# kallenordling/cesm_emulator

Measured on NVIDIA B200. Metric: train samples/s (baseline cfg), higher is better.
Workload: dtype fp16

## Files before the change

### cesm_emulator_b200/_lib.py

```python
from __future__ import annotations

import ctypes
from ctypes import POINTER, Structure, c_char_p, c_float, c_int32, c_int64, c_void_p
from pathlib import Path

_PKG = Path(__file__).resolve().parent
_VARIANT = __import__("os").environ.get("CESM_LIB_VARIANT", "")
LIB_PATH = _PKG / (f"libcesm_b200_{_VARIANT}.so" if _VARIANT else "libcesm_b200.so")

CESM_MAX_TAPS = 16


class IgemmArgs(Structure):

    _fields_ = [
        ("a0", c_void_p), ("a1", c_void_p),
        ("c0", c_int32), ("c1", c_int32),
        ("n", c_int32), ("h", c_int32), ("w", c_int32),
        ("stride", c_int32),
        ("num_taps", c_int32),
        ("tap_dh", c_int32 * CESM_MAX_TAPS), ("tap_dw", c_int32 * CESM_MAX_TAPS),
        ("wt", c_void_p), ("cout", c_int32),
        ("oh", c_int32), ("ow", c_int32),
        ("out", c_void_p), ("out_fp32", c_int32), ("ldo", c_int32),
# ... 68 lines not shown
    _lib = lib
    return lib


_P, _I, _L, _F = c_void_p, ctypes.c_int, ctypes.c_longlong, c_float
_SIGNATURES: dict[str, list] = {
    "cesm_igemm": [POINTER(IgemmArgs), _P],
    "cesm_wgrad": [POINTER(WgradArgs), _P],
    "cesm_pack_weight": [_P, _P, _I, _I, _I, _L, _L, POINTER(c_int32), _P],
    "cesm_pack_weights_batched": [_P, _I, _P],
    "cesm_unpack_wgrads_batched": [_P, _I, _P],
    "cesm_unpack_wgrad": [_P, _P, _I, _I, _I, _L, _L, POINTER(c_int32), _I, _P],
    "cesm_adamw_step": [_P, _P, _P, _P, _L, _P, _P, _F, _F, _F, _F, _P],
    "cesm_colsum": [_P, _P, _L, _I, _I, _P],
    "cesm_gn_stats": [_P, _P, _I, _L, _I, _I, _P],
    "cesm_gn_apply_fwd": [_P, _P, _P, _P, _P, _P, _P, _I, _L, _I, _I, _F, _P],
    "cesm_gn_bwd": [_P, _P, _P, _P, _P, _P, _P, _P, _P, _P, _P, _P, _I, _L, _I, _I, _F, _I, _P],
    "cesm_ln_fwd": [_P, _P, _P, _L, _I, _F, _P],
    "cesm_ln_bwd": [_P, _P, _P, _P, _P, _P, _L, _I, _F, _I, _P],
    "cesm_tattn_fwd": [_P, _P, _P, _P, _P, _P, _I, _I, _I, _I, _I, _F, _P],
    "cesm_tattn_bwd": [_P, _P, _P, _P, _P, _P, _P, _P, _P, _I, _I, _I, _I, _I, _F, _P],
    "cesm_tattn_proj_fwd": [_P, _P, _P, _P, _P, _P, _I, _I, _I, _I, _I, _I, _F, _P],
    "cesm_tattn_proj_bwd": [_P, _P, _P, _P, _P, _P, _P, _P, _I, _I, _I, _I, _I, _I, _F, _P],
    "cesm_tattn_long_fwd": [_P, _P, _P, _P, _P, _P, _I, _I, _I, _I, _I, _F, _P],
    "cesm_tattn_long_bwd": [_P, _P, _P, _P, _P, _P, _P, _P, _P, _I, _I, _I, _I, _I, _F, _P],
    "cesm_mattn_fwd": [_P, _P, _P, _I, _I, _I, _I, _F, _P],
    "cesm_mattn_bwd": [_P, _P, _P, _P, _P, _P, _I, _I, _I, _I, _F, _P],
    "cesm_linattn_fwd": [_P, _P, _P, _I, _I, _I, _I, _F, _P],
    "cesm_linattn_fwd_out": [_P, _P, _P, _P, _P, _P, _I, _I, _I, _I, _I, _F, _P],
    "cesm_linattn_bwd": [_P, _P, _P, _P, _P, _I, _I, _I, _I, _F, _P],
    "cesm_film_fwd": [_P, _P, _P, _I, _I, _I, _I, _P],
    "cesm_film_bwd": [_P, _P, _P, _I, _I, _P, _I, _I, _I, _P],
    "cesm_gather_windows": [_P, _P, _P, _P, _P, _I, _I, _I, _I, _I, _I, _I, _I, _P],
    "cesm_qkv_bwd": [_P, _P, _P, _P, _P, _L, _L, _I, _I, _P],
    "cesm_input_patches": [_P, _P, _I, _I, _P, _I, _I, _I, _I, _I, _I, _P],
    "cesm_input_weight_pack": [_P, _P, _P, _I, _I, _I, _P],
    "cesm_input_conv_fwd": [_P, _P, _I, _I, _P, _P, _P, _I, _I, _I, _I, _I, _I, _P],
    "cesm_input_conv_wgrad": [_P, _P, _I, _I, _P, _P, _P, _I, _I, _I, _I, _I, _I, _P],
    "cesm_out_conv_fwd": [_P, _P, _P, _P, _I, _I, _I, _L, _I, _P],
    "cesm_out_conv_bwd": [_P, _P, _P, _P, _P, _P, _I, _I, _I, _L, _I, _P],
    "cesm_sinusoidal": [_P, _P, _I, _I, _P],
    "cesm_small_linear_fwd": [_P, _P, _P, _P, _I, _I, _I, _I, _P],
    "cesm_small_linear_bwd": [_P, _P, _P, _P, _P, _P, _I, _I, _I, _I, _I, _P],
    "cesm_q_sample": [_P, _P, _P, _P, _P, _P, _I, _L, _P],
    "cesm_mse_fwd": [_P, _P, _P, _P, _L, _P],
    "cesm_scale_by_scalar": [_P, _P, _F, _P, _L, _P],
# ... 76 lines not shown
```

### cesm_emulator_b200/csrc/api_common.h

```cpp
#pragma once
#include <cuda.h>
#include <cuda_runtime.h>
#include <stdarg.h>
#include <stdint.h>

#include "../../include/cesm_b200.h"

namespace cesm {

int set_error(int code, const char* fmt, ...);
#define CESM_CHECK_CUDA(expr)                                                                  \
    do {                                                                                       \
        cudaError_t _e = (expr);                                                               \
        if (_e != cudaSuccess)                                                                 \
            return ::cesm::set_error(CESM_ERR_CUDA, "%s failed: %s (%s:%d)", #expr,            \
                                     cudaGetErrorString(_e), __FILE__, __LINE__);              \
    } while (0)
void note_launch();
#define CESM_CHECK_LAUNCH()            \
    do {                               \
        ::cesm::note_launch();         \
        CESM_CHECK_CUDA(cudaGetLastError()); \
    } while (0)
bool scratch_prezeroed();
// ... 30 lines not shown
    cfg.blockDim = block;
    cfg.dynamicSmemBytes = smem;
    cfg.stream = st;
    cudaLaunchAttribute attr[2];
    int n = 0;
    if (pdl_enabled()) {
        attr[n].id = cudaLaunchAttributeProgrammaticStreamSerialization;
        attr[n].val.programmaticStreamSerializationAllowed = 1;
        ++n;
    }
    if (cluster_x > 1) {
        attr[n].id = cudaLaunchAttributeClusterDimension;
        attr[n].val.clusterDim.x = (unsigned)cluster_x;
        attr[n].val.clusterDim.y = 1;
        attr[n].val.clusterDim.z = 1;
        ++n;
    }
    cfg.attrs = attr;
    cfg.numAttrs = n;
    return cudaLaunchKernelEx(&cfg, kern, static_cast<KArgs>(args)...);
}

int get_tensor_map_h16(CUtensorMap* out, const void* base, int rank, const uint64_t* dims,
                        const uint64_t* strides_bytes, const uint32_t* box);

inline cudaStream_t as_stream(void* s) { return reinterpret_cast<cudaStream_t>(s); }
inline int ceil_div(int a, int b) { return (a + b - 1) / b; }

}
```

### cesm_emulator_b200/csrc/api_core.cu

```cuda
#include <stdlib.h>

#include <atomic>
#include <mutex>
#include <string>
#include <unordered_map>

#include "api_common.h"
#include "igemm.h"

namespace cesm {

static thread_local std::string g_last_error;
static std::atomic<long long> g_launches{0};
void note_launch() { g_launches.fetch_add(1, std::memory_order_relaxed); }
bool pdl_enabled() {
    static const bool on = [] { const char* e = getenv("CESM_NO_PDL"); return !(e && atoi(e)); }();
    return on;
}
static std::atomic<int> g_prezeroed{0};
bool scratch_prezeroed() { return g_prezeroed.load(std::memory_order_relaxed) != 0; }

int set_error(int code, const char* fmt, ...) {
    char buf[1024];
    va_list ap;
// ... 2 lines not shown
    va_end(ap);
    g_last_error = buf;
    return code;
}

typedef CUresult (*EncodeTiledFn)(CUtensorMap*, CUtensorMapDataType, cuuint32_t, void*, const cuuint64_t*,
                                  const cuuint64_t*, const cuuint32_t*, const cuuint32_t*, CUtensorMapInterleave,
                                  CUtensorMapSwizzle, CUtensorMapL2promotion, CUtensorMapFloatOOBfill);

static EncodeTiledFn resolve_encode() {
    static EncodeTiledFn fn = nullptr;
    static std::once_flag once;
    std::call_once(once, [] {
        void* p = nullptr;
        cudaDriverEntryPointQueryResult q;
        if (cudaGetDriverEntryPoint("cuTensorMapEncodeTiled", &p, cudaEnableDefault, &q) == cudaSuccess &&
            q == cudaDriverEntryPointSuccess)
            fn = reinterpret_cast<EncodeTiledFn>(p);
    });
    return fn;
}

struct MapKey {
    uint64_t v[14];
    bool operator==(const MapKey& o) const {
        for (int i = 0; i < 14; ++i)
            if (v[i] != o.v[i]) return false;
        return true;
    }
};
struct MapKeyHash {
    size_t operator()(const MapKey& k) const {
        uint64_t h = 1469598103934665603ull;
        for (int i = 0; i < 14; ++i) {
            h ^= k.v[i];
            h *= 1099511628211ull;
        }
        return static_cast<size_t>(h);
    }
};
static std::mutex g_map_mutex;
static std::unordered_map<MapKey, CUtensorMap, MapKeyHash> g_map_cache;

int get_tensor_map_h16(CUtensorMap* out, const void* base, int rank, const uint64_t* dims,
                        const uint64_t* strides_bytes, const uint32_t* box) {
    CESM_REQUIRE(rank >= 2 && rank <= 4, "tensor map rank %d unsupported", rank);
    CESM_REQUIRE((reinterpret_cast<uintptr_t>(base) & 15u) == 0, "tensor base %p not 16-byte aligned", base);
    MapKey key{};
    key.v[0] = reinterpret_cast<uint64_t>(base);
    key.v[1] = static_cast<uint64_t>(rank);
    for (int i = 0; i < rank; ++i) {
        key.v[2 + i] = dims[i];
        key.v[6 + i] = (i == 0) ? 0 : strides_bytes[i - 1];
        key.v[10 + i] = box[i];
    }
    {
        std::lock_guard<std::mutex> lk(g_map_mutex);
        auto it = g_map_cache.find(key);
        if (it != g_map_cache.end()) {
            *out = it->second;
            return CESM_OK;
        }
    }
    EncodeTiledFn enc = resolve_encode();
    if (!enc) return set_error(CESM_ERR_CUDA, "cuTensorMapEncodeTiled unavailable (no CUDA driver?)");
    cuuint64_t gdim[4], gstr[3];
    cuuint32_t bx[4], es[4];
    for (int i = 0; i < rank; ++i) {
        gdim[i] = dims[i];
        bx[i] = box[i];
        es[i] = 1;
        if (i > 0) {
            gstr[i - 1] = strides_bytes[i - 1];
            CESM_REQUIRE(gstr[i - 1] % 16 == 0, "tensor map stride %llu not a multiple of 16 B",
                         (unsigned long long)gstr[i - 1]);
        }
        CESM_REQUIRE(bx[i] >= 1 && bx[i] <= 256, "tensor map box[%d]=%u out of range", i, bx[i]);
    }
    alignas(64) CUtensorMap m;
    CUresult r = enc(&m, CU_TENSOR_MAP_DATA_TYPE_FLOAT16, rank, const_cast<void*>(base), gdim, gstr, bx, es,
                     CU_TENSOR_MAP_INTERLEAVE_NONE, CU_TENSOR_MAP_SWIZZLE_128B, CU_TENSOR_MAP_L2_PROMOTION_L2_256B,
                     CU_TENSOR_MAP_FLOAT_OOB_FILL_NONE);
    if (r != CUDA_SUCCESS) return set_error(CESM_ERR_CUDA, "cuTensorMapEncodeTiled failed with CUresult %d", (int)r);
    {
        std::lock_guard<std::mutex> lk(g_map_mutex);
        if (g_map_cache.size() > 8192) g_map_cache.clear();
        g_map_cache.emplace(key, m);
    }
    *out = m;
    return CESM_OK;
}

static void choose_tile(int n, int oh, int ow, int* bw, int* bh, int* bn) {
    long long best_tiles = -1;
    int b_w = 1, b_h = 1, b_n = 1;
    for (int w = 1; w <= 128 && w <= ow; ++w) {
        if (!(w == ow || (w & (w - 1)) == 0)) continue;
        for (int h = 1; h * w <= 128 && h <= oh; ++h) {
            if (!(h == oh || (h & (h - 1)) == 0)) continue;
            int nn = 128 / (w * h);
            if (nn > n) nn = n;
            if (nn < 1) nn = 1;
            if (w != ow || h != oh) nn = 1;
            long long tiles = 1LL * ceil_div(ow, w) * ceil_div(oh, h) * ceil_div(n, nn);
// ... 584 lines not shown
```

### cesm_emulator_b200/kernels.py

```python
from __future__ import annotations

import ctypes
from typing import Optional, Sequence, Tuple

import torch

from . import _lib
from ._lib import IgemmArgs

H16 = torch.float16


def _stream() -> ctypes.c_void_p:
    return ctypes.c_void_p(torch.cuda.current_stream().cuda_stream)


def _ptr(t: Optional[torch.Tensor]) -> Optional[int]:
    return None if t is None else t.data_ptr()


def _req_cuda(*ts: Optional[torch.Tensor]) -> None:
    for t in ts:
        if t is not None and not t.is_cuda:
            raise _lib.CesmError("cesm_emulator_b200 kernels need CUDA tensors (no CPU fallback)")
# ... 339 lines not shown

def tattn_proj_fwd(xn, wqkv_packed, bias, cs, sn, B: int, F: int, HW: int, H: int, D: int, scale: float):
    _req_cuda(xn, wqkv_packed, bias, cs, sn)
    assert xn.dtype == H16 and wqkv_packed.dtype == H16 and tuple(wqkv_packed.shape) == (3 * H * D, 64)
    rows = B * F * HW
    out = torch.empty((rows, H * D), dtype=H16, device=xn.device)
    _lib.call("cesm_tattn_proj_fwd", _ptr(xn), _ptr(wqkv_packed), _ptr(bias), _ptr(cs), _ptr(sn), _ptr(out), B, F, HW, H, D,
              64, scale, _stream(),
              _meta={"kind": "fused", "flops": 2.0 * rows * 64 * 3 * H * D, "bytes": float(rows * (64 + H * D) * 2)})
    return out


def tattn_proj_bwd(xn, wqkv_packed, bias, cs, sn, dout, B: int, F: int, HW: int, H: int, D: int, scale: float):
    _req_cuda(xn, wqkv_packed, bias, cs, sn, dout)
    rows = B * F * HW
    dqkv = torch.empty((rows, 3 * H * D), dtype=H16, device=xn.device)
    dbias = zero_scratch((H, F, F), xn.device)
    _lib.call("cesm_tattn_proj_bwd", _ptr(xn), _ptr(wqkv_packed), _ptr(bias), _ptr(cs), _ptr(sn), _ptr(dout), _ptr(dqkv),
              _ptr(dbias), B, F, HW, H, D, 64, scale, _stream(),
              _meta={"kind": "fused", "flops": 2.0 * rows * 64 * 3 * H * D, "bytes": float(rows * (64 + H * D + 3 * H * D) * 2)})
    return dqkv, dbias


def mattn_fwd(qkv, NI: int, n: int, H: int, D: int, scale: float):
    _req_cuda(qkv)
    assert qkv.dtype == H16 and qkv.shape == (NI * n, 3 * H * D), (tuple(qkv.shape), NI, n, H, D)
    out = torch.empty((NI * n, H * D), dtype=H16, device=qkv.device)
    lse = torch.empty((NI * n, H), dtype=torch.float32, device=qkv.device)
    _lib.call("cesm_mattn_fwd", _ptr(qkv), _ptr(out), _ptr(lse), NI, n, H, D, scale, _stream(),
              _meta={"kind": "fwd", "flops": 4.0 * NI * H * n * n * D, "bytes": float(qkv.numel() * 2 + out.numel() * 2)})
    return out, lse


def mattn_bwd(qkv, out, lse, dout, NI: int, n: int, H: int, D: int, scale: float):
    _req_cuda(qkv, out, lse, dout)
    assert qkv.dtype == H16 and out.dtype == H16 and dout.dtype == H16 and lse.dtype == torch.float32
    assert qkv.shape == (NI * n, 3 * H * D) and out.shape == dout.shape == (NI * n, H * D) and lse.numel() == NI * n * H
    dqkv = torch.empty_like(qkv)
    delta = torch.empty((NI * n, H), dtype=torch.float32, device=qkv.device)
    _lib.call("cesm_mattn_bwd", _ptr(qkv), _ptr(out), _ptr(lse), _ptr(dout), _ptr(dqkv), _ptr(delta), NI, n, H, D, scale,
              _stream(), _meta={"kind": "bwd", "flops": 14.0 * NI * H * n * n * D,
                                "bytes": float(qkv.numel() * 4 + out.numel() * 2 + dout.numel() * 2)})
    return dqkv


def linattn_fwd(qkv, NI: int, n: int, H: int, D: int, scale: float):
# ... 208 lines not shown
```

### cesm_emulator_b200/ops.py

```python
from __future__ import annotations

import weakref
from typing import Optional, Tuple

import torch

from . import _lib
from . import kernels as K

H16 = torch.float16

_PHASE_TAPS = {0: [(0, 1), (-1, 3)], 1: [(1, 0), (0, 2)]}


_OUTER_GRAD = [True]


class _Fn(torch.autograd.Function):
    @classmethod
    def apply(cls, *args, **kwargs):
        _OUTER_GRAD[0] = torch.is_grad_enabled()
        return super().apply(*args, **kwargs)


# ... 570 lines not shown
        dxn, dw = K.qkv_bwd(dqkv4, xn, wdq)
        return dxn, dw.view_as(wqkv)
    return K.igemm(dqkv4, wdq), _conv_wgrad(wqkv, xn, None, dqkv4, 1)


class TemporalAttnBlockFn(_Fn):

    @staticmethod
    def forward(ctx, x, gamma, wqkv, wout, pos_bias, cs, sn, B, F, meta):
        x = x.contiguous()
        NI, H_, W_, C = x.shape
        heads, D, eps = meta.heads, meta.dim_head, meta.eps
        hidden = heads * D
        g = gamma.reshape(-1)
        pos_bias = pos_bias.contiguous().float()
        train = _train(ctx)
        if F == 1 and not train and C == 64:
            wln, colsum = _fold_f1(meta, wqkv, wout, hidden, C, gamma=gamma)
            return K.igemm(x, wln, residual=x, ln_fold=(colsum, eps))
        xn = K.ln_fwd(x, g, eps)
        if F == 1 and not train:
            return K.igemm(xn, _fold_f1(meta, wqkv, wout, hidden, C), residual=x)
        wq = _conv_fwd_weight(meta.cq, wqkv, 3 * hidden, C, 1, train)
        fused = K.tattn_proj_ok(C, F, H_ * W_, heads, D, train)
        if fused:
            qkv, lse = None, None
            o = K.tattn_proj_fwd(xn.view(-1, C), wq, pos_bias, cs, sn, B, F, H_ * W_, heads, D, D ** -0.5)
        else:
            qkv = K.igemm(xn, wq)
            o, lse = K.tattn_fwd(qkv.view(-1, 3 * hidden), pos_bias, cs, sn, B, F, H_ * W_, heads, D, D ** -0.5)
        y = K.igemm(o.view(NI, H_, W_, hidden), _conv_fwd_weight(meta.co, wout, C, hidden, 1, train), residual=x)
        ctx.wdq = _conv_dgrad_weights(meta.cq, wqkv, 3 * hidden, C, 0, 1, train)[0]
        ctx.wdo = _conv_dgrad_weights(meta.co, wout, C, hidden, 0, 1, train)[0]
        ctx.wq_fwd = wq if fused else None
        saved = [x, g, xn, o, pos_bias, cs, sn, wqkv, wout, gamma]
        if not fused:
            saved.append(qkv)
            if F > 4:
                saved.append(lse)
        ctx.save_for_backward(*saved)
        ctx.cfg, ctx.gshape = (B, F, heads, D, eps), gamma.shape
        return y

    @staticmethod
    def backward(ctx, dy):
        saved = ctx.saved_tensors
        x, g, xn, o, pos_bias, cs, sn, wqkv, wout, gamma = saved[:10]
        qkv = saved[10] if len(saved) > 10 else None
        lse = saved[11] if len(saved) > 11 else None
        B, F, heads, D, eps = ctx.cfg
        hidden = heads * D
        NI, H_, W_, C = x.shape
        dy = dy.contiguous()
        do = K.igemm(dy, ctx.wdo)
        dwout = _conv_wgrad(wout, o.view(NI, H_, W_, hidden), None, dy, 1)
        if ctx.wq_fwd is not None:
            dqkv, dbias = K.tattn_proj_bwd(xn.view(-1, C), ctx.wq_fwd, pos_bias, cs, sn, do.view(-1, hidden), B, F, H_ * W_,
                                           heads, D, D ** -0.5)
        else:
            dqkv, dbias = K.tattn_bwd(qkv.view(-1, 3 * hidden), pos_bias, cs, sn, o if F > 4 else None, lse,
                                      do.view(-1, hidden), B, F, H_ * W_, heads, D, D ** -0.5)
        dqkv4 = dqkv.view(NI, H_, W_, 3 * hidden)
        dxn, dwqkv = _qkv_backward(wqkv, ctx.wdq, xn, dqkv4)
        if _direct_all(gamma):
            dx, _ = K.ln_bwd(x, g, dxn, dy, eps, into=gamma.grad.view(-1))
            _ready(gamma)
            dgamma = None
        else:
            dx, dg = K.ln_bwd(x, g, dxn, dy, eps)
            dgamma = dg.view(ctx.gshape)
        return dx, dgamma, dwqkv, dwout, dbias, None, None, None, None, None


class MidAttnBlockFn(_Fn):

    @staticmethod
    def forward(ctx, x, gamma, wqkv, wout, meta):
        x = x.contiguous()
        NI, H_, W_, C = x.shape
# ... 226 lines not shown
```

### include/cesm_b200.h

```cpp
#ifndef CESM_B200_H
#define CESM_B200_H

#include <stddef.h>
#include <stdint.h>

#ifdef __cplusplus
extern "C" {
#endif

typedef enum cesm_status {
    CESM_OK = 0,
    CESM_ERR_INVALID = -1,
    CESM_ERR_CUDA = -2,
    CESM_ERR_INTERNAL = -3
} cesm_status;

const char* cesm_last_error(void);
const char* cesm_version(void);
long long cesm_launch_count(void);


#define CESM_MAX_TAPS 16

typedef struct cesm_igemm_args {
// ... 73 lines not shown
int cesm_gn_stats(const void* x, float* sums, int B, long long P, int C, int G, void* stream);
int cesm_gn_apply_fwd(const void* x, const float* sums, const float* gamma, const float* beta, const float* film,
                      const void* residual, void* out, int B, long long P, int C, int G, float eps, void* stream);
int cesm_gn_bwd(const void* x, const void* dout, const float* sums, const float* gamma, const float* beta,
                const float* film, float* csum, void* dx, float* dgamma, float* dbeta, float* dfilm,
                float* dconv_bias, int B, long long P, int C, int G, float eps, int accumulate_params, void* stream);

int cesm_ln_fwd(const void* x, const float* gamma, void* out, long long M, int C, float eps, void* stream);
int cesm_ln_bwd(const void* x, const float* gamma, const void* dy, const void* dres, void* dx, float* dgamma,
                long long M, int C, float eps, int accumulate, void* stream);

int cesm_tattn_fwd(const void* qkv, const float* bias, const float* cs, const float* sn, void* out, float* lse,
                   int B, int F, int HW, int H, int dim_head, float scale, void* stream);
int cesm_tattn_bwd(const void* qkv, const float* bias, const float* cs, const float* sn, const void* out,
                   const float* lse, const void* dout, void* dqkv, float* dbias, int B, int F, int HW, int H,
                   int dim_head, float scale, void* stream);

int cesm_tattn_proj_fwd(const void* xn, const void* wqkv, const float* bias, const float* cs, const float* sn, void* out,
                        int B, int F, int HW, int H, int dim_head, int cin, float scale, void* stream);
int cesm_tattn_proj_bwd(const void* xn, const void* wqkv, const float* bias, const float* cs, const float* sn,
                        const void* dout, void* dqkv, float* dbias, int B, int F, int HW, int H, int dim_head, int cin,
                        float scale, void* stream);

int cesm_tattn_long_max_frames(void);
int cesm_tattn_long_fwd(const void* qkv, const float* bias_diag, const float* cs, const float* sn, void* out,
                        float* lse, int B, int F, int HW, int H, int dim_head, float scale, void* stream);
int cesm_tattn_long_bwd(const void* qkv, const float* bias_diag, const float* cs, const float* sn, const void* out,
                        const float* lse, const void* dout, void* dqkv, float* dbias_diag, int B, int F, int HW, int H,
                        int dim_head, float scale, void* stream);

int cesm_mattn_fwd(const void* qkv, void* out, float* lse, int NI, int n, int H, int dim_head, float scale, void* stream);
int cesm_mattn_bwd(const void* qkv, const void* out, const float* lse, const void* dout, void* dqkv, float* delta, int NI,
                   int n, int H, int dim_head, float scale, void* stream);

size_t cesm_linattn_ws_floats(int NI, int H);
int cesm_linattn_fwd(const void* qkv, float* ws, void* out, int NI, int n, int H, int dim_head, float scale,
                     void* stream);
int cesm_linattn_fwd_out(const void* qkv, float* ws, const float* wout, const float* bias, const void* x, void* y, int NI,
                         int n, int H, int dim_head, int C, float scale, void* stream);
int cesm_linattn_bwd(const void* qkv, float* ws, const void* dout, float* scratch, void* dqkv, int NI, int n, int H,
                     int dim_head, float scale, void* stream);

typedef struct cesm_film_desc {
    const float* W;
    const float* bias;
    float* dW;
// ... 43 lines not shown
```

Measured before the change: 188.3.

## Add tcgen05/UMMA fused QKV-projection temporal attention kernels for training

Adds a new warp-specialized Blackwell kernel that computes the QKV projection with tcgen05 UMMA into tensor memory, then applies RoPE, small-frame softmax attention and writes output via TMA, with a matching backward that also accumulates the bias gradient. Training temporal attention with C=64, 8 heads, dim 32 and up to 3 frames now routes here instead of the existing fused proj path. The goal is to remove the separate QKV materialization and use tensor cores for the projection. Tensor map creation gains a 64B swizzle option and the map cache key grows to include it. The new pipeline is complex, and correctness or occupancy depends on the large shared-memory footprint and the 512-column TMEM allocation.

```diff
diff --git a/cesm_emulator_b200/_lib.py b/cesm_emulator_b200/_lib.py
--- a/cesm_emulator_b200/_lib.py
+++ b/cesm_emulator_b200/_lib.py
@@ -114,6 +114,8 @@
     "cesm_tattn_bwd": [_P, _P, _P, _P, _P, _P, _P, _P, _P, _I, _I, _I, _I, _I, _F, _P],
     "cesm_tattn_proj_fwd": [_P, _P, _P, _P, _P, _P, _I, _I, _I, _I, _I, _I, _F, _P],
     "cesm_tattn_proj_bwd": [_P, _P, _P, _P, _P, _P, _P, _P, _I, _I, _I, _I, _I, _I, _F, _P],
+    "cesm_tattn_umma_fwd": [_P, _P, _P, _P, _P, _P, _I, _I, _I, _I, _I, _I, _F, _P],
+    "cesm_tattn_umma_bwd": [_P, _P, _P, _P, _P, _P, _P, _P, _I, _I, _I, _I, _I, _I, _F, _P],
     "cesm_tattn_long_fwd": [_P, _P, _P, _P, _P, _P, _I, _I, _I, _I, _I, _F, _P],
     "cesm_tattn_long_bwd": [_P, _P, _P, _P, _P, _P, _P, _P, _P, _I, _I, _I, _I, _I, _F, _P],
     "cesm_mattn_fwd": [_P, _P, _P, _I, _I, _I, _I, _F, _P],
diff --git a/cesm_emulator_b200/csrc/api_common.h b/cesm_emulator_b200/csrc/api_common.h
--- a/cesm_emulator_b200/csrc/api_common.h
+++ b/cesm_emulator_b200/csrc/api_common.h
@@ -76,7 +76,7 @@
 }
 
 int get_tensor_map_h16(CUtensorMap* out, const void* base, int rank, const uint64_t* dims,
-                        const uint64_t* strides_bytes, const uint32_t* box);
+                        const uint64_t* strides_bytes, const uint32_t* box, int swizzle_bytes = 128);
 
 inline cudaStream_t as_stream(void* s) { return reinterpret_cast<cudaStream_t>(s); }
 inline int ceil_div(int a, int b) { return (a + b - 1) / b; }
diff --git a/cesm_emulator_b200/csrc/api_core.cu b/cesm_emulator_b200/csrc/api_core.cu
--- a/cesm_emulator_b200/csrc/api_core.cu
+++ b/cesm_emulator_b200/csrc/api_core.cu
@@ -48,9 +48,9 @@
 }
 
 struct MapKey {
-    uint64_t v[14];
+    uint64_t v[15];
     bool operator==(const MapKey& o) const {
-        for (int i = 0; i < 14; ++i)
+        for (int i = 0; i < 15; ++i)
             if (v[i] != o.v[i]) return false;
         return true;
     }
@@ -58,7 +58,7 @@
 struct MapKeyHash {
     size_t operator()(const MapKey& k) const {
         uint64_t h = 1469598103934665603ull;
-        for (int i = 0; i < 14; ++i) {
+        for (int i = 0; i < 15; ++i) {
             h ^= k.v[i];
             h *= 1099511628211ull;
         }
@@ -69,8 +69,9 @@
 static std::unordered_map<MapKey, CUtensorMap, MapKeyHash> g_map_cache;
 
 int get_tensor_map_h16(CUtensorMap* out, const void* base, int rank, const uint64_t* dims,
-                        const uint64_t* strides_bytes, const uint32_t* box) {
+                        const uint64_t* strides_bytes, const uint32_t* box, int swizzle_bytes) {
     CESM_REQUIRE(rank >= 2 && rank <= 4, "tensor map rank %d unsupported", rank);
+    CESM_REQUIRE(swizzle_bytes == 128 || swizzle_bytes == 64, "tensor map swizzle %d unsupported", swizzle_bytes);
     CESM_REQUIRE((reinterpret_cast<uintptr_t>(base) & 15u) == 0, "tensor base %p not 16-byte aligned", base);
     MapKey key{};
     key.v[0] = reinterpret_cast<uint64_t>(base);
@@ -80,6 +81,7 @@
         key.v[6 + i] = (i == 0) ? 0 : strides_bytes[i - 1];
         key.v[10 + i] = box[i];
     }
+    key.v[14] = static_cast<uint64_t>(swizzle_bytes);
     {
         std::lock_guard<std::mutex> lk(g_map_mutex);
         auto it = g_map_cache.find(key);
@@ -105,7 +107,8 @@
     }
     alignas(64) CUtensorMap m;
     CUresult r = enc(&m, CU_TENSOR_MAP_DATA_TYPE_FLOAT16, rank, const_cast<void*>(base), gdim, gstr, bx, es,
-                     CU_TENSOR_MAP_INTERLEAVE_NONE, CU_TENSOR_MAP_SWIZZLE_128B, CU_TENSOR_MAP_L2_PROMOTION_L2_256B,
+                     CU_TENSOR_MAP_INTERLEAVE_NONE,
+                     swizzle_bytes == 64 ? CU_TENSOR_MAP_SWIZZLE_64B : CU_TENSOR_MAP_SWIZZLE_128B, CU_TENSOR_MAP_L2_PROMOTION_L2_256B,
                      CU_TENSOR_MAP_FLOAT_OOB_FILL_NONE);
     if (r != CUDA_SUCCESS) return set_error(CESM_ERR_CUDA, "cuTensorMapEncodeTiled failed with CUresult %d", (int)r);
     {
diff --git a/cesm_emulator_b200/csrc/tattn_umma.cu b/cesm_emulator_b200/csrc/tattn_umma.cu
--- /dev/null
+++ b/cesm_emulator_b200/csrc/tattn_umma.cu
@@ -0,0 +1,660 @@
+#include "api_common.h"
+#include "common.cuh"
+
+namespace cesm {
+namespace tu {
+
+static constexpr int C = 64, D = 32, HEADS = 8, HID = HEADS * D, TILE = 128;
+static constexpr int XT = TILE * C * 2;
+static constexpr int WPART = D * C * 2;
+static constexpr int WS = 3 * WPART;
+static constexpr int DOT = TILE * D * 2;
+static constexpr int STT = 32 * D * 2;
+static constexpr int EPI = 256;
+static constexpr uint32_t TM_V = 384;
+
+template <int F, bool BWD>
+struct Cfg {
+    static constexpr int XST = BWD ? 1 : 2;
+    static constexpr int NST = BWD ? 3 * F : F;
+    static constexpr int W_OFF = XST * F * XT;
+    static constexpr int DO_OFF = W_OFF + 2 * WS;
+    static constexpr int ST_OFF = DO_OFF + (BWD ? F * DOT : 0);
+    static constexpr int XB_OFF = ST_OFF + 4 * NST * STT;
+    static constexpr int DB_OFF = XB_OFF + 2 * F * F * TILE * 4;
+    static constexpr int TAB_OFF = DB_OFF + (BWD ? HEADS * F * F * TILE * 4 : 0);
+    static constexpr int BAR_OFF = (TAB_OFF + (2 * F * 16 + HEADS * F * F) * 4 + 7) & ~7;
+    static constexpr int SMEM = 1024 + BAR_OFF + 17 * 8;
+};
+
+struct Maps {
+    CUtensorMap x;
+    CUtensorMap w;
+    CUtensorMap o;
+    CUtensorMap g;
+};
+struct Params {
+    int HW, tiles_per_img, items;
+    float scale;
+    const float* bias;
+    const float* cs;
+    const float* sn;
+    float* dbias;
+};
+
+__device__ __forceinline__ void tma_load_3d(uint32_t dst, const void* map, uint32_t bar, int c0, int c1, int c2) {
+    asm volatile(
+        "cp.async.bulk.tensor.3d.shared::cluster.global.mbarrier::complete_tx::bytes [%0], [%1, {%3, %4, %5}], [%2];"
+        :
+        : "r"(dst), "l"(reinterpret_cast<uint64_t>(map)), "r"(bar), "r"(c0), "r"(c1), "r"(c2)
+        : "memory");
+}
+__device__ __forceinline__ void tma_store_3d(const void* map, uint32_t src, int c0, int c1, int c2) {
+    asm volatile("cp.async.bulk.tensor.3d.global.shared::cta.bulk_group [%0, {%2, %3, %4}], [%1];"
+                 :
+                 : "l"(reinterpret_cast<uint64_t>(map)), "r"(src), "r"(c0), "r"(c1), "r"(c2)
+                 : "memory");
+}
+__device__ __forceinline__ void bulk_commit() { asm volatile("cp.async.bulk.commit_group;" ::: "memory"); }
+__device__ __forceinline__ void bulk_wait_read0() { asm volatile("cp.async.bulk.wait_group.read 0;" ::: "memory"); }
+__device__ __forceinline__ void tmem_ld16(uint32_t taddr, float (&f)[16]) {
+    asm volatile(
+        "tcgen05.ld.sync.aligned.32x32b.x16.b32 "
+        "{%0, %1, %2, %3, %4, %5, %6, %7, %8, %9, %10, %11, %12, %13, %14, %15}, [%16];"
+        : "=f"(f[0]), "=f"(f[1]), "=f"(f[2]), "=f"(f[3]), "=f"(f[4]), "=f"(f[5]), "=f"(f[6]), "=f"(f[7]), "=f"(f[8]),
+          "=f"(f[9]), "=f"(f[10]), "=f"(f[11]), "=f"(f[12]), "=f"(f[13]), "=f"(f[14]), "=f"(f[15])
+        : "r"(taddr)
+        : "memory");
+}
+__device__ __forceinline__ void tmem_ld16(uint32_t taddr, float (&f)[8]) {
+    asm volatile("tcgen05.ld.sync.aligned.32x32b.x8.b32 {%0, %1, %2, %3, %4, %5, %6, %7}, [%8];"
+                 : "=f"(f[0]), "=f"(f[1]), "=f"(f[2]), "=f"(f[3]), "=f"(f[4]), "=f"(f[5]), "=f"(f[6]), "=f"(f[7])
+                 : "r"(taddr)
+                 : "memory");
+}
+template <int N>
+__device__ __forceinline__ void tmem_fence(float (&f)[N]) {
+#pragma unroll
+    for (int i = 0; i < N; ++i) asm volatile("" : "+f"(f[i]));
+}
+__device__ __forceinline__ void sts128(uint32_t addr, uint32_t a, uint32_t b, uint32_t c, uint32_t d) {
+    asm volatile("st.shared.v4.b32 [%0], {%1, %2, %3, %4};" ::"r"(addr), "r"(a), "r"(b), "r"(c), "r"(d) : "memory");
+}
+__device__ __forceinline__ uint4 lds128(uint32_t addr) {
+    uint4 u;
+    asm volatile("ld.shared.v4.b32 {%0, %1, %2, %3}, [%4];"
+                 : "=r"(u.x), "=r"(u.y), "=r"(u.z), "=r"(u.w)
+                 : "r"(addr)
+                 : "memory");
+    return u;
+}
+__device__ __forceinline__ uint32_t sw64(int r, int c) { return r * 64 + ((c ^ ((r >> 1) & 3)) << 4); }
+template <int N>
+__device__ __forceinline__ void put16(uint32_t tile, int r, int c, const float (&f)[N]) {
+#pragma unroll
+    for (int u = 0; u < N / 8; ++u)
+        sts128(tile + sw64(r, (N / 8) * c + u), pack_h2(f[8 * u + 0], f[8 * u + 1]), pack_h2(f[8 * u + 2], f[8 * u + 3]),
+               pack_h2(f[8 * u + 4], f[8 * u + 5]), pack_h2(f[8 * u + 6], f[8 * u + 7]));
+}
+template <int N>
+__device__ __forceinline__ void unpack16(const uint32_t* u, int c, float (&f)[N]) {
+#pragma unroll
+    for (int i = 0; i < N / 2; ++i) {
+        const float2 t = unpack_h2(u[(N / 2) * c + i]);
+        f[2 * i] = t.x;
+        f[2 * i + 1] = t.y;
+    }
+}
+template <int N>
+__device__ __forceinline__ void rope16(float (&f)[N], const float* cs, const float* sn, float scale) {
+#pragma unroll
+    for (int m = 0; m < N / 2; ++m) {
+        const float x0 = f[2 * m] * scale, x1 = f[2 * m + 1] * scale;
+        f[2 * m] = x0 * cs[m] - x1 * sn[m];
+        f[2 * m + 1] = x1 * cs[m] + x0 * sn[m];
+    }
+}
+template <int N>
+__device__ __forceinline__ void rope16_t(float (&f)[N], const float* cs, const float* sn, float scale) {
+#pragma unroll
+    for (int m = 0; m < N / 2; ++m) {
+        const float g0 = f[2 * m], g1 = f[2 * m + 1];
+        f[2 * m] = (g0 * cs[m] + g1 * sn[m]) * scale;
+        f[2 * m + 1] = (g1 * cs[m] - g0 * sn[m]) * scale;
+    }
+}
+template <int N>
+__device__ __forceinline__ float dot16(const float (&a)[N], const float (&b)[N]) {
+    float s = 0.f;
+#pragma unroll
+    for (int i = 0; i < N; ++i) s = fmaf(a[i], b[i], s);
+    return s;
+}
+__device__ __forceinline__ void epi_sync() { asm volatile("bar.sync 5, %0;" ::"n"(EPI) : "memory"); }
+__device__ __forceinline__ void pair_sync(int q) { asm volatile("bar.sync %0, 64;" ::"r"(q + 1) : "memory"); }
+template <int N>
+__device__ __forceinline__ void pair_sum(float (&v)[N], float* xb, int r, int q, int half) {
+    if (half)
+#pragma unroll
+        for (int k = 0; k < N; ++k) xb[k * TILE + r] = v[k];
+    pair_sync(q);
+    if (!half)
+#pragma unroll
+        for (int k = 0; k < N; ++k) {
+            v[k] += xb[k * TILE + r];
+            xb[k * TILE + r] = v[k];
+        }
+    pair_sync(q);
+    if (half)
+#pragma unroll
+        for (int k = 0; k < N; ++k) v[k] = xb[k * TILE + r];
+}
+
+template <int F>
+__device__ __forceinline__ void scores(uint32_t tq, int c2, const float* cs_s, const float* sn_s, float scale, float* s) {
+#pragma unroll
+    for (int i = 0; i < F * F; ++i) s[i] = 0.f;
+#pragma unroll
+    for (int sub = 0; sub < 2; ++sub) {
+        const int c4 = 2 * c2 + sub;
+        float q[F][8], k[F][8];
+#pragma unroll
+        for (int f = 0; f < F; ++f) {
+            tmem_ld16(tq + f * 64 + c4 * 8, q[f]);
+            tmem_ld16(tq + f * 64 + 32 + c4 * 8, k[f]);
+        }
+        tmem_ld_wait();
+#pragma unroll
+        for (int f = 0; f < F; ++f) {
+            tmem_fence(q[f]);
+            tmem_fence(k[f]);
+            rope16(q[f], cs_s + f * 16 + c4 * 4, sn_s + f * 16 + c4 * 4, scale);
+            rope16(k[f], cs_s + f * 16 + c4 * 4, sn_s + f * 16 + c4 * 4, 1.f);
+        }
+#pragma unroll
+        for (int i = 0; i < F; ++i)
+#pragma unroll
+            for (int j = 0; j < F; ++j) s[i * F + j] += dot16(q[i], k[j]);
+    }
+}
+
+template <int F>
+__device__ __forceinline__ void softmax(float* s, const float* bias_s, int h) {
+#pragma unroll
+    for (int i = 0; i < F; ++i) {
+        float m = -INFINITY;
+#pragma unroll
+        for (int j = 0; j < F; ++j) {
+            s[i * F + j] += bias_s[(h * F + i) * F + j];
+            m = fmaxf(m, s[i * F + j]);
+        }
+        float l = 0.f;
+#pragma unroll
+        for (int j = 0; j < F; ++j) {
+            s[i * F + j] = __expf(s[i * F + j] - m);
+            l += s[i * F + j];
+        }
+        const float inv = 1.f / l;
+#pragma unroll
+        for (int j = 0; j < F; ++j) s[i * F + j] *= inv;
+    }
+}
+
+template <int F, bool BWD>
+__device__ __forceinline__ void tattn_umma_body(const Maps& maps, const Params& p) {
+    using K = Cfg<F, BWD>;
+    extern __shared__ uint8_t smem_raw[];
+    const uint32_t smem_base = (smem_u32(smem_raw) + 1023u) & ~1023u;
+    uint8_t* smem_gen = smem_raw + (smem_base - smem_u32(smem_raw));
+    const uint32_t x_base = smem_base, w_base = smem_base + K::W_OFF, do_base = smem_base + K::DO_OFF;
+    const uint32_t bar_base = smem_base + K::BAR_OFF;
+    auto x_full = [&](int s) { return bar_base + 8u * s; };
+    auto x_empty = [&](int s) { return bar_base + 8u * (2 + s); };
+    auto w_full = [&](int s) { return bar_base + 8u * (4 + s); };
+    auto w_empty = [&](int s) { return bar_base + 8u * (6 + s); };
+    auto qk_full = [&](int s) { return bar_base + 8u * (8 + s); };
+    auto qk_empty = [&](int s) { return bar_base + 8u * (10 + s); };
+    const uint32_t v_full = bar_base + 8u * 12, v_empty = bar_base + 8u * 13;
+    const uint32_t do_full = bar_base + 8u * 14, do_empty = bar_base + 8u * 15;
+    const uint32_t tmem_ptr_addr = bar_base + 8u * 16;
+    volatile uint32_t* tmem_ptr_gen = reinterpret_cast<volatile uint32_t*>(smem_gen + (tmem_ptr_addr - smem_base));
+    float* cs_s = reinterpret_cast<float*>(smem_gen + K::TAB_OFF);
+    float* sn_s = cs_s + F * 16;
+    float* bias_s = sn_s + F * 16;
+    float* db_s = reinterpret_cast<float*>(smem_gen + K::DB_OFF);
+    float* xb_s = reinterpret_cast<float*>(smem_gen + K::XB_OFF);
+
+    const int warp = threadIdx.x >> 5, lane = threadIdx.x & 31;
+    if (threadIdx.x == 0) {
+        tma_prefetch_desc(&maps.x);
+        tma_prefetch_desc(&maps.w);
+        tma_prefetch_desc(&maps.o);
+        if (BWD) tma_prefetch_desc(&maps.g);
+        for (int s = 0; s < 2; ++s) {
+            mbar_init(x_full(s), 1);
+            mbar_init(x_empty(s), 1);
+            mbar_init(w_full(s), 1);
+            mbar_init(w_empty(s), 1);
+            mbar_init(qk_full(s), 1);
+            mbar_init(qk_empty(s), 8);
+        }
+        mbar_init(v_full, 1);
+        mbar_init(v_empty, 8);
+        mbar_init(do_full, 1);
+        mbar_init(do_empty, 8);
+        fence_barrier_init();
+    }
+    if (warp == 8) tmem_alloc(tmem_ptr_addr, 512);
+    pdl_wait();
+    for (int i = threadIdx.x; i < F * 16; i += blockDim.x) {
+        cs_s[i] = p.cs[i];
+        sn_s[i] = p.sn[i];
+    }
+    for (int i = threadIdx.x; i < HEADS * F * F; i += blockDim.x) bias_s[i] = p.bias[i];
+    if (BWD)
+        for (int i = threadIdx.x; i < HEADS * F * F * TILE; i += blockDim.x) db_s[i] = 0.f;
+    tc_fence_before();
+    __syncthreads();
+    tc_fence_after();
+    const uint32_t tmem_base = *tmem_ptr_gen;
+
+    if (warp == 8) {
+        if (elect_one()) {
+            int xs = 0, ws = 0;
+            uint32_t xph = 0, wph = 0, dph = 0;
+            for (int item = blockIdx.x; item < p.items; item += gridDim.x) {
+                const int b = item / p.tiles_per_img, hw0 = (item % p.tiles_per_img) * TILE;
+                mbar_wait(x_empty(xs), xph ^ 1u, 60);
+                mbar_arrive_expect_tx(x_full(xs), F * XT);
+#pragma unroll
+                for (int f = 0; f < F; ++f) tma_load_3d(x_base + (xs * F + f) * XT, &maps.x, x_full(xs), 0, hw0, b * F + f);
+                if (++xs == K::XST) {
+                    xs = 0;
+                    xph ^= 1u;
+                }
+                for (int h = 0; h < HEADS; ++h) {
+                    mbar_wait(w_empty(ws), wph ^ 1u, 61);
+                    mbar_arrive_expect_tx(w_full(ws), WS);
+#pragma unroll
+                    for (int part = 0; part < 3; ++part)
+                        tma_load_2d(w_base + ws * WS + part * WPART, &maps.w, w_full(ws), 0, part * HID + h * D);
+                    if (++ws == 2) {
+                        ws = 0;
+                        wph ^= 1u;
+                    }
+                    if (BWD) {
+                        mbar_wait(do_empty, dph ^ 1u, 62);
+                        mbar_arrive_expect_tx(do_full, F * DOT);
+#pragma unroll
+                        for (int f = 0; f < F; ++f) tma_load_3d(do_base + f * DOT, &maps.g, do_full, h * D, hw0, b * F + f);
+                        dph ^= 1u;
+                    }
+                }
+            }
+        }
+        __syncwarp();
+    } else if (warp == 9) {
+        constexpr uint32_t idesc = make_idesc_f16(TILE, D, 0, 0);
+        if (elect_one()) {
+            const uint64_t dk = make_smem_desc_sw128(0, 0, 1024);
+            int xs = 0, ws = 0, qs = 0;
+            uint32_t xph = 0, wph = 0, qph = 0, vph = 0;
+            for (int item = blockIdx.x; item < p.items; item += gridDim.x) {
+                mbar_wait(x_full(xs), xph, 63);
+                tc_fence_after();
+                for (int h = 0; h < HEADS; ++h) {
+                    mbar_wait(w_full(ws), wph, 64);
+                    tc_fence_after();
+                    const uint32_t w16 = (w_base + ws * WS) >> 4;
+                    auto mma = [&](uint32_t d, int f, int part) {
+                        const uint32_t a16 = (x_base + (xs * F + f) * XT) >> 4, b16 = w16 + part * (WPART >> 4);
+#pragma unroll
+                        for (int k = 0; k < 4; ++k)
+                            umma_f16(d, dk | (uint64_t)(a16 + 2 * k), dk | (uint64_t)(b16 + 2 * k), idesc, k ? 1u : 0u);
+                    };
+                    auto issue_qk = [&]() {
+                        mbar_wait(qk_empty(qs), qph ^ 1u, 65);
+                        tc_fence_after();
+#pragma unroll
+                        for (int f = 0; f < F; ++f) {
+                            mma(tmem_base + qs * 192 + f * 64, f, 0);
+                            mma(tmem_base + qs * 192 + f * 64 + 32, f, 1);
+                        }
+                        umma_commit(qk_full(qs));
+                        if (++qs == 2) {
+                            qs = 0;
+                            qph ^= 1u;
+                        }
+                    };
+                    auto issue_v = [&]() {
+                        mbar_wait(v_empty, vph ^ 1u, 66);
+                        tc_fence_after();
+#pragma unroll
+                        for (int f = 0; f < F; ++f) mma(tmem_base + TM_V + f * 32, f, 2);
+                        umma_commit(v_full);
+                        vph ^= 1u;
+                    };
+                    if (BWD) {
+                        issue_v();
+                        issue_qk();
+                    } else {
+                        issue_qk();
+                        issue_v();
+                    }
+                    umma_commit(w_empty(ws));
+                    if (++ws == 2) {
+                        ws = 0;
+                        wph ^= 1u;
+                    }
+                }
+                umma_commit(x_empty(xs));
+                if (++xs == K::XST) {
+                    xs = 0;
+                    xph ^= 1u;
+                }
+            }
+        }
+        __syncwarp();
+    } else {
+        const int q = warp & 3, half = warp >> 2;
+        const int r = q * 32 + lane;
+        const bool issuer = half == 0 && lane == 0;
+        const uint32_t lane_base = static_cast<uint32_t>(q * 32) << 16;
+        const uint32_t st_base = smem_base + K::ST_OFF + q * K::NST * STT;
+        int qs = 0;
+        uint32_t qph = 0, vph = 0, dph = 0;
+        for (int item = blockIdx.x; item < p.items; item += gridDim.x) {
+            const int b = item / p.tiles_per_img, hw0 = (item % p.tiles_per_img) * TILE;
+            const bool valid = hw0 + r < p.HW;
+            const bool store = issuer && hw0 + q * 32 < p.HW;
+            for (int h = 0; h < HEADS; ++h) {
+                const uint32_t tq = tmem_base + lane_base + qs * 192, tv = tmem_base + lane_base + TM_V;
+                if constexpr (!BWD) {
+                    float pr[F * F];
+                    mbar_wait(qk_full(qs), qph, 67);
+                    tc_fence_after();
+                    scores<F>(tq, half, cs_s, sn_s, p.scale, pr);
+                    tc_fence_before();
+                    __syncwarp();
+                    if (lane == 0) mbar_arrive(qk_empty(qs));
+                    if (issuer) bulk_wait_read0();
+                    __syncwarp();
+                    pair_sum(pr, xb_s, r, q, half);
+                    softmax<F>(pr, bias_s, h);
+                    mbar_wait(v_full, vph, 68);
+                    tc_fence_after();
+                    float v[F][16];
+#pragma unroll
+                    for (int f = 0; f < F; ++f) tmem_ld16(tv + f * 32 + half * 16, v[f]);
+                    tmem_ld_wait();
+#pragma unroll
+                    for (int f = 0; f < F; ++f) tmem_fence(v[f]);
+                    tc_fence_before();
+                    __syncwarp();
+                    if (lane == 0) mbar_arrive(v_empty);
+                    vph ^= 1u;
+#pragma unroll
+                    for (int i = 0; i < F; ++i) {
+                        float o[16];
+#pragma unroll
+                        for (int e = 0; e < 16; ++e) o[e] = 0.f;
+#pragma unroll
+                        for (int j = 0; j < F; ++j)
+#pragma unroll
+                            for (int e = 0; e < 16; ++e) o[e] = fmaf(pr[i * F + j], v[j][e], o[e]);
+                        put16(st_base + i * STT, lane, half, o);
+                    }
+                    fence_proxy_async();
+                    pair_sync(q);
+                    if (store) {
+#pragma unroll
+                        for (int i = 0; i < F; ++i) tma_store_3d(&maps.o, st_base + i * STT, h * D, hw0 + q * 32, b * F + i);
+                        bulk_commit();
+                    }
+                } else {
+                    uint32_t g[F][8];
+                    mbar_wait(do_full, dph, 69);
+#pragma unroll
+                    for (int f = 0; f < F; ++f)
+#pragma unroll
+                        for (int c = 0; c < 2; ++c) {
+                            const uint4 u = lds128(do_base + f * DOT + sw64(r, 2 * half + c));
+                            g[f][4 * c + 0] = u.x;
+                            g[f][4 * c + 1] = u.y;
+                            g[f][4 * c + 2] = u.z;
+                            g[f][4 * c + 3] = u.w;
+                        }
+                    dph ^= 1u;
+                    float sd[2 * F * F];
+                    mbar_wait(v_full, vph, 70);
+                    tc_fence_after();
+                    {
+                        float v[F][16];
+#pragma unroll
+                        for (int f = 0; f < F; ++f) tmem_ld16(tv + f * 32 + half * 16, v[f]);
+                        tmem_ld_wait();
+#pragma unroll
+                        for (int f = 0; f < F; ++f) tmem_fence(v[f]);
+                        tc_fence_before();
+                        __syncwarp();
+                        if (lane == 0) mbar_arrive(v_empty);
+                        vph ^= 1u;
+#pragma unroll
+                        for (int i = 0; i < F; ++i) {
+                            float go[16];
+                            unpack16(g[i], 0, go);
+#pragma unroll
+                            for (int j = 0; j < F; ++j) sd[F * F + i * F + j] = dot16(go, v[j]);
+                        }
+                    }
+                    __syncwarp();
+                    if (lane == 0) mbar_arrive(do_empty);
+                    mbar_wait(qk_full(qs), qph, 71);
+                    tc_fence_after();
+                    scores<F>(tq, half, cs_s, sn_s, p.scale, sd);
+                    if (issuer) bulk_wait_read0();
+                    __syncwarp();
+                    pair_sum(sd, xb_s, r, q, half);
+                    float* pr = sd;
+                    float* dp = sd + F * F;
+                    softmax<F>(pr, bias_s, h);
+#pragma unroll
+                    for (int i = 0; i < F; ++i) {
+                        float di = 0.f;
+#pragma unroll
+                        for (int j = 0; j < F; ++j) di = fmaf(pr[i * F + j], dp[i * F + j], di);
+#pragma unroll
+                        for (int j = 0; j < F; ++j) {
+                            dp[i * F + j] = pr[i * F + j] * (dp[i * F + j] - di);
+                            if (valid && !half) db_s[((h * F + i) * F + j) * TILE + r] += dp[i * F + j];
+                        }
+                    }
+#pragma unroll
+                    for (int cl = 0; cl < 2; ++cl) {
+                        const int c4 = 2 * half + cl;
+                        const float* cf = cs_s + c4 * 4;
+                        const float* sf = sn_s + c4 * 4;
+                        float qv[F][8], kv[F][8];
+#pragma unroll
+                        for (int f = 0; f < F; ++f) {
+                            tmem_ld16(tq + f * 64 + c4 * 8, qv[f]);
+                            tmem_ld16(tq + f * 64 + 32 + c4 * 8, kv[f]);
+                        }
+                        tmem_ld_wait();
+#pragma unroll
+                        for (int f = 0; f < F; ++f) {
+                            tmem_fence(qv[f]);
+                            tmem_fence(kv[f]);
+                            rope16(qv[f], cf + f * 16, sf + f * 16, p.scale);
+                            rope16(kv[f], cf + f * 16, sf + f * 16, 1.f);
+                        }
+#pragma unroll
+                        for (int f = 0; f < F; ++f) {
+                            float t[8];
+#pragma unroll
+                            for (int e = 0; e < 8; ++e) t[e] = 0.f;
+#pragma unroll
+                            for (int j = 0; j < F; ++j)
+#pragma unroll
+                                for (int e = 0; e < 8; ++e) t[e] = fmaf(dp[f * F + j], kv[j][e], t[e]);
+                            rope16_t(t, cf + f * 16, sf + f * 16, p.scale);
+                            put16(st_base + (3 * f + 0) * STT, lane, c4, t);
+#pragma unroll
+                            for (int e = 0; e < 8; ++e) t[e] = 0.f;
+#pragma unroll
+                            for (int i = 0; i < F; ++i)
+#pragma unroll
+                                for (int e = 0; e < 8; ++e) t[e] = fmaf(dp[i * F + f], qv[i][e], t[e]);
+                            rope16_t(t, cf + f * 16, sf + f * 16, 1.f);
+                            put16(st_base + (3 * f + 1) * STT, lane, c4, t);
+#pragma unroll
+                            for (int e = 0; e < 8; ++e) t[e] = 0.f;
+#pragma unroll
+                            for (int i = 0; i < F; ++i) {
+                                float go[8];
+                                unpack16(g[i], cl, go);
+#pragma unroll
+                                for (int e = 0; e < 8; ++e) t[e] = fmaf(pr[i * F + f], go[e], t[e]);
+                            }
+                            put16(st_base + (3 * f + 2) * STT, lane, c4, t);
+                        }
+                    }
+                    tc_fence_before();
+                    fence_proxy_async();
+                    __syncwarp();
+                    if (lane == 0) mbar_arrive(qk_empty(qs));
+                    pair_sync(q);
+                    if (store) {
+#pragma unroll
+                        for (int f = 0; f < F; ++f)
+#pragma unroll
+                            for (int part = 0; part < 3; ++part)
+                                tma_store_3d(&maps.o, st_base + (3 * f + part) * STT, part * HID + h * D, hw0 + q * 32,
+                                             b * F + f);
+                        bulk_commit();
+                    }
+                }
+                if (++qs == 2) {
+                    qs = 0;
+                    qph ^= 1u;
+                }
+            }
+        }
+        if (issuer) bulk_wait_read0();
+        if (BWD) {
+            epi_sync();
+            const int et = threadIdx.x;
+            for (int i = et; i < HEADS * F * F; i += EPI) {
+                float s = 0.f;
+                for (int t = 0; t < TILE; ++t) s += db_s[i * TILE + t];
+                atomicAdd(p.dbias + i, s);
+            }
+        }
+    }
+    tc_fence_before();
+    __syncthreads();
+    if (warp == 8) tmem_dealloc(tmem_base, 512);
+}
+
+template <int F>
+__global__ void __launch_bounds__(EPI + 64, 1) tattn_umma_fwd_kernel(const __grid_constant__ Maps maps, const Params p) {
+    pdl_trigger();
+    tattn_umma_body<F, false>(maps, p);
+}
+template <int F>
+__global__ void __launch_bounds__(EPI + 64, 1) tattn_umma_bwd_kernel(const __grid_constant__ Maps maps, const Params p) {
+    pdl_trigger();
+    tattn_umma_body<F, true>(maps, p);
+}
+
+static int check(int B, int F, int HW, int H, int dim_head, int cin) {
+    CESM_REQUIRE(cin == C, "tattn_umma needs 64 input channels (got %d)", cin);
+    CESM_REQUIRE(F >= 1 && F <= 3, "tattn_umma needs 1 <= F <= 3 frames (got %d)", F);
+    CESM_REQUIRE(H == HEADS && dim_head == D, "tattn_umma needs 8 heads of 32 (got %d x %d)", H, dim_head);
+    CESM_REQUIRE(B >= 1 && HW >= 1, "bad B=%d HW=%d", B, HW);
+    return CESM_OK;
+}
+
+static int map3(CUtensorMap* m, const void* base, int width, int HW, int BF, uint32_t box0, uint32_t box1, int swz) {
+    const uint64_t dims[3] = {(uint64_t)width, (uint64_t)HW, (uint64_t)BF};
+    const uint64_t str[2] = {(uint64_t)width * 2, (uint64_t)width * 2 * HW};
+    const uint32_t box[3] = {box0, box1, 1u};
+    return get_tensor_map_h16(m, base, 3, dims, str, box, swz);
+}
+
+template <int F, bool BWD, typename Kern>
+static int launch(Kern kern, const Maps& maps, Params p, int B, void* stream) {
+    p.tiles_per_img = (p.HW + TILE - 1) / TILE;
+    p.items = B * p.tiles_per_img;
+    static bool cfg = false;
+    if (!cfg) {
+        CESM_CHECK_CUDA(cudaFuncSetAttribute(kern, cudaFuncAttributeMaxDynamicSharedMemorySize, Cfg<F, BWD>::SMEM));
+        cfg = true;
+    }
+    int sms = 148, dev = 0;
+    if (cudaGetDevice(&dev) == cudaSuccess) cudaDeviceGetAttribute(&sms, cudaDevAttrMultiProcessorCount, dev);
+    const int grid = p.items < sms ? p.items : sms;
+    launch_pdl(kern, grid, EPI + 64, Cfg<F, BWD>::SMEM, as_stream(stream), maps, p);
+    CESM_CHECK_LAUNCH();
+    return CESM_OK;
+}
+
+}
+}
+
+using namespace cesm;
+
+extern "C" int cesm_tattn_umma_fwd(const void* xn, const void* wqkv, const float* bias, const float* cs, const float* sn,
+                                   void* out, int B, int F, int HW, int H, int dim_head, int cin, float scale, void* stream) {
+    if (int rc = tu::check(B, F, HW, H, dim_head, cin)) return rc;
+    tu::Maps maps;
+    if (int rc = tu::map3(&maps.x, xn, tu::C, HW, B * F, tu::C, tu::TILE, 128)) return rc;
+    {
+        const uint64_t dims[2] = {(uint64_t)tu::C, (uint64_t)(3 * tu::HID)};
+        const uint64_t str[1] = {(uint64_t)tu::C * 2};
+        const uint32_t box[2] = {(uint32_t)tu::C, (uint32_t)tu::D};
+        if (int rc = get_tensor_map_h16(&maps.w, wqkv, 2, dims, str, box)) return rc;
+    }
+    if (int rc = tu::map3(&maps.o, out, tu::HID, HW, B * F, tu::D, 32, 64)) return rc;
+    maps.g = maps.o;
+    tu::Params p{};
+    p.HW = HW;
+    p.scale = scale;
+    p.bias = bias;
+    p.cs = cs;
+    p.sn = sn;
+    switch (F) {
+        case 1: return tu::launch<1, false>(tu::tattn_umma_fwd_kernel<1>, maps, p, B, stream);
+        case 2: return tu::launch<2, false>(tu::tattn_umma_fwd_kernel<2>, maps, p, B, stream);
+        default: return tu::launch<3, false>(tu::tattn_umma_fwd_kernel<3>, maps, p, B, stream);
+    }
+}
+
+extern "C" int cesm_tattn_umma_bwd(const void* xn, const void* wqkv, const float* bias, const float* cs, const float* sn,
+                                   const void* dout, void* dqkv, float* dbias, int B, int F, int HW, int H, int dim_head,
+                                   int cin, float scale, void* stream) {
+    if (int rc = tu::check(B, F, HW, H, dim_head, cin)) return rc;
+    tu::Maps maps;
+    if (int rc = tu::map3(&maps.x, xn, tu::C, HW, B * F, tu::C, tu::TILE, 128)) return rc;
+    {
+        const uint64_t dims[2] = {(uint64_t)tu::C, (uint64_t)(3 * tu::HID)};
+        const uint64_t str[1] = {(uint64_t)tu::C * 2};
+        const uint32_t box[2] = {(uint32_t)tu::C, (uint32_t)tu::D};
+        if (int rc = get_tensor_map_h16(&maps.w, wqkv, 2, dims, str, box)) return rc;
+    }
+    if (int rc = tu::map3(&maps.o, dqkv, 3 * tu::HID, HW, B * F, tu::D, 32, 64)) return rc;
+    if (int rc = tu::map3(&maps.g, dout, tu::HID, HW, B * F, tu::D, tu::TILE, 64)) return rc;
+    CESM_ZERO_SCRATCH(dbias, sizeof(float) * H * F * F, as_stream(stream));
+    tu::Params p{};
+    p.HW = HW;
+    p.scale = scale;
+    p.bias = bias;
+    p.cs = cs;
+    p.sn = sn;
+    p.dbias = dbias;
+    switch (F) {
+        case 1: return tu::launch<1, true>(tu::tattn_umma_bwd_kernel<1>, maps, p, B, stream);
+        case 2: return tu::launch<2, true>(tu::tattn_umma_bwd_kernel<2>, maps, p, B, stream);
+        default: return tu::launch<3, true>(tu::tattn_umma_bwd_kernel<3>, maps, p, B, stream);
+    }
+}
diff --git a/cesm_emulator_b200/kernels.py b/cesm_emulator_b200/kernels.py
--- a/cesm_emulator_b200/kernels.py
+++ b/cesm_emulator_b200/kernels.py
@@ -385,6 +385,40 @@
     return dqkv, dbias
 
 
+def tattn_umma_ok(C: int, F: int, H: int, D: int, train: bool) -> bool:
+    return train and not _FUSED_TATTN_TRAIN and C == 64 and 1 <= F <= 3 and H == 8 and D == 32
+
+
+def _umma_flops(rows: int, F: int, H: int, D: int) -> float:
+    return 2.0 * rows * 64 * 3 * H * D + 4.0 * rows * H * F * D
+
+
+def tattn_umma_fwd(xn, wqkv_packed, bias, cs, sn, B: int, F: int, HW: int, H: int, D: int, scale: float):
+    _req_cuda(xn, wqkv_packed, bias, cs, sn)
+    assert xn.dtype == H16 and wqkv_packed.dtype == H16 and tuple(wqkv_packed.shape) == (3 * H * D, 64)
+    rows = B * F * HW
+    assert xn.numel() == rows * 64
+    out = torch.empty((rows, H * D), dtype=H16, device=xn.device)
+    _lib.call("cesm_tattn_umma_fwd", _ptr(xn), _ptr(wqkv_packed), _ptr(bias), _ptr(cs), _ptr(sn), _ptr(out), B, F, HW, H, D,
+              64, scale, _stream(),
+              _meta={"kind": "umma", "flops": _umma_flops(rows, F, H, D), "bytes": float(rows * (64 + H * D) * 2)})
+    return out
+
+
+def tattn_umma_bwd(xn, wqkv_packed, bias, cs, sn, dout, B: int, F: int, HW: int, H: int, D: int, scale: float):
+    _req_cuda(xn, wqkv_packed, bias, cs, sn, dout)
+    assert xn.dtype == H16 and dout.dtype == H16 and tuple(wqkv_packed.shape) == (3 * H * D, 64)
+    rows = B * F * HW
+    assert xn.numel() == rows * 64 and dout.numel() == rows * H * D
+    dqkv = torch.empty((rows, 3 * H * D), dtype=H16, device=xn.device)
+    dbias = zero_scratch((H, F, F), xn.device)
+    flops = 2.0 * rows * 64 * 3 * H * D + 10.0 * rows * H * F * D
+    _lib.call("cesm_tattn_umma_bwd", _ptr(xn), _ptr(wqkv_packed), _ptr(bias), _ptr(cs), _ptr(sn), _ptr(dout), _ptr(dqkv),
+              _ptr(dbias), B, F, HW, H, D, 64, scale, _stream(),
+              _meta={"kind": "umma", "flops": flops, "bytes": float(rows * (64 + H * D + 3 * H * D) * 2)})
+    return dqkv, dbias
+
+
 def mattn_fwd(qkv, NI: int, n: int, H: int, D: int, scale: float):
     _req_cuda(qkv)
     assert qkv.dtype == H16 and qkv.shape == (NI * n, 3 * H * D), (tuple(qkv.shape), NI, n, H, D)
diff --git a/cesm_emulator_b200/ops.py b/cesm_emulator_b200/ops.py
--- a/cesm_emulator_b200/ops.py
+++ b/cesm_emulator_b200/ops.py
@@ -616,8 +616,12 @@
         if F == 1 and not train:
             return K.igemm(xn, _fold_f1(meta, wqkv, wout, hidden, C), residual=x)
         wq = _conv_fwd_weight(meta.cq, wqkv, 3 * hidden, C, 1, train)
-        fused = K.tattn_proj_ok(C, F, H_ * W_, heads, D, train)
-        if fused:
+        umma = K.tattn_umma_ok(C, F, heads, D, train)
+        fused = umma or K.tattn_proj_ok(C, F, H_ * W_, heads, D, train)
+        if umma:
+            qkv, lse = None, None
+            o = K.tattn_umma_fwd(xn.view(-1, C), wq, pos_bias, cs, sn, B, F, H_ * W_, heads, D, D ** -0.5)
+        elif fused:
             qkv, lse = None, None
             o = K.tattn_proj_fwd(xn.view(-1, C), wq, pos_bias, cs, sn, B, F, H_ * W_, heads, D, D ** -0.5)
         else:
@@ -627,6 +631,7 @@
         ctx.wdq = _conv_dgrad_weights(meta.cq, wqkv, 3 * hidden, C, 0, 1, train)[0]
         ctx.wdo = _conv_dgrad_weights(meta.co, wout, C, hidden, 0, 1, train)[0]
         ctx.wq_fwd = wq if fused else None
+        ctx.umma = umma
         saved = [x, g, xn, o, pos_bias, cs, sn, wqkv, wout, gamma]
         if not fused:
             saved.append(qkv)
@@ -648,7 +653,10 @@
         dy = dy.contiguous()
         do = K.igemm(dy, ctx.wdo)
         dwout = _conv_wgrad(wout, o.view(NI, H_, W_, hidden), None, dy, 1)
-        if ctx.wq_fwd is not None:
+        if ctx.umma:
+            dqkv, dbias = K.tattn_umma_bwd(xn.view(-1, C), ctx.wq_fwd, pos_bias, cs, sn, do.view(-1, hidden), B, F, H_ * W_,
+                                           heads, D, D ** -0.5)
+        elif ctx.wq_fwd is not None:
             dqkv, dbias = K.tattn_proj_bwd(xn.view(-1, C), ctx.wq_fwd, pos_bias, cs, sn, do.view(-1, hidden), B, F, H_ * W_,
                                            heads, D, D ** -0.5)
         else:
diff --git a/include/cesm_b200.h b/include/cesm_b200.h
--- a/include/cesm_b200.h
+++ b/include/cesm_b200.h
@@ -119,6 +119,12 @@
                         const void* dout, void* dqkv, float* dbias, int B, int F, int HW, int H, int dim_head, int cin,
                         float scale, void* stream);
 
+int cesm_tattn_umma_fwd(const void* xn, const void* wqkv, const float* bias, const float* cs, const float* sn, void* out,
+                        int B, int F, int HW, int H, int dim_head, int cin, float scale, void* stream);
+int cesm_tattn_umma_bwd(const void* xn, const void* wqkv, const float* bias, const float* cs, const float* sn,
+                        const void* dout, void* dqkv, float* dbias, int B, int F, int HW, int H, int dim_head, int cin,
+                        float scale, void* stream);
+
 int cesm_tattn_long_max_frames(void);
 int cesm_tattn_long_fwd(const void* qkv, const float* bias_diag, const float* cs, const float* sn, void* out,
                         float* lse, int B, int F, int HW, int H, int dim_head, float scale, void* stream);
```

After: 198.7 (median of 6 runs). 1.06x the previous value.
